# kkahatapitiya/Coarse-Fine-Networks

Hardware: AMD Instinct MI355X
Metric: clips/sec (fwd+bwd+SGD) x3d_fine X3D-M T=256x224x224 (higher is better)
Workload: dtype f32; 1 GPU; x3d_fine X3D-M train step (fwd+loss+bwd+SGD), 8x3x256x224x224 clips per GPU, random-init weights; clips_per_gpu=8, frames=256, parallelism=dp1, launch=eager

## Files before the change

### coarse-fine-networks_amd/cfn_hip/ops.py

```python
import torch
from torch.autograd import Function
from torch.autograd.function import once_differentiable

import ctypes
import threading

from . import call, call_try, check, query, ACT_NONE, ACT_RELU, ACT_SWISH, ACT_SIGMOID


_scratch_epoch = [0]


class _ZeroArena(object):
    CHUNK = 1 << 20

    def __init__(self):
        self.buf, self.off, self.epoch = {}, {}, _scratch_epoch[0]

    def take(self, numel, dev):
        if self.epoch != _scratch_epoch[0]:
            self.buf, self.off, self.epoch = {}, {}, _scratch_epoch[0]
        numel_al = (numel + 1) & ~1
        key = (dev.type, dev.index)
        if key not in self.buf or self.off[key] + numel_al > self.buf[key].numel():
            self.buf[key] = torch.zeros(max(self.CHUNK, numel_al), dtype=torch.float64, device=dev)
            self.off[key] = 0
        o = self.off[key]
        self.off[key] = o + numel_al
        return self.buf[key][o:o + numel]


class _GradCast(object):

    def __init__(self):
        self._reset()
        self.last_total = 0

    def _reset(self):
        self.cur, self.live, self.scheduled, self.seen, self.task = {}, [], False, set(), None

    def begin(self):
        tid = torch._C._current_graph_task_id()
        if tid != self.task:
            if self.live:
                self.flush()
            self._reset()
            self.task = tid

    def first_use(self, w):
        if id(w) in self.seen:
            return False
        self.seen.add(id(w))
        return True

    def take(self, numel, shape, dev):
        al = (numel + 3) & ~3
        key = (dev.type, dev.index)
        ch = self.cur.get(key)
        if ch is None or ch['off'] + al > ch['f64'].numel():
            size = max(int(self.last_total * 1.05) + 1024, al, 1 << 16)
            ch = {'f64': torch.zeros(size, dtype=torch.float64, device=dev),
                  'f32': torch.empty(size, dtype=torch.float32, device=dev), 'off': 0, 'done': 0}
            self.cur[key] = ch
            self.live.append(ch)
        o = ch['off']
        ch['off'] = o + al
        if not self.scheduled:
            torch.autograd.Variable._execution_engine.queue_callback(self._end_of_backward)
            self.scheduled = True
        return ch['f64'][o:o + numel], ch['f32'][o:o + numel].view(shape)

    def flush(self):
        for ch in self.live:
            if ch['off'] > ch['done']:
                ch['f32'][ch['done']:ch['off']].copy_(ch['f64'][ch['done']:ch['off']])
                ch['done'] = ch['off']

    def _end_of_backward(self):
        self.flush()
        self.last_total = max(sum(ch['off'] for ch in self.live), 1)
        self._reset()


class _PerThread(threading.local):

    def __init__(self):
        self.arena = _ZeroArena()
        self.gradcast = _GradCast()


_tls = _PerThread()
LAZY_GRAD_CAST = True


def _f64(n, c, dev):
    return _tls.arena.take(n * c, dev).view(n, c)


def _f64pair(n, c, dev):
    t = _tls.arena.take(2 * n * c, dev).view(2, n, c)
    return t, t[0], t[1]


def reset_scratch():
    _scratch_epoch[0] += 1


def flush_grad_casts():
    _tls.gradcast.flush()


def allow_lazy_grad_cast(params, ok=True):
    for p in params:
        p._cfn_lazy_grad_ok = bool(ok)


def _lazy_ok(w):
    if not LAZY_GRAD_CAST or w is None or not w.is_leaf or w.grad is not None or torch.is_grad_enabled():
        return False
    if not getattr(w, '_cfn_lazy_grad_ok', False):
        return False
    if w._backward_hooks:
        return False
    hooks = getattr(w, '_post_accumulate_grad_hooks', None)
    if hooks:
        from .dist import _BucketHook
        if not all(isinstance(h, _BucketHook) for h in hooks.values()):
            return False
    return True


def _lazy_ok_probe(w):
    with torch.no_grad():
        return _lazy_ok(w)


def _grad_owner(w):
    if w is not None and not w.is_leaf and w._is_view():
        base = w._base
        if base is not None and base.is_leaf and base.numel() == w.numel() and w.is_contiguous() and base.is_contiguous():
            return base
    return w


def _gw_buffers(w, rows, cols, dev):
    gc = _tls.gradcast
    owner = _grad_owner(w)
    if _lazy_ok(owner):
        gc.begin()
        if gc.first_use(owner):
            g64, g32 = gc.take(rows * cols, tuple(w.shape), dev)
            return g64.view(rows, cols), (lambda: g32)
        gc.flush()
    g64 = _f64(rows, cols, dev)
    return g64, (lambda: g64.float().view(tuple(w.shape)))


def _opt(t):
    return None if t is None else t.contiguous()


def _coef(t, rows=None, cols=None):
    if t is None:
        return None
    if rows is not None and t.numel() != rows * cols:
        raise RuntimeError('per-sample coefficients of %d x %d channels expected, got a tensor of shape %s' % (rows, cols, tuple(t.shape)))
    return t.to(torch.float64).contiguous()


class ShortcutToken(object):

    def __init__(self):
        self.acc, self.acc_stride, self.main_done = None, 1, False


class TailLink(object):

    def __init__(self):
        self.y_scale = self.res_scale = None
        self.done = False


def _bf(t):
    return t is not None and t.dtype in (torch.bfloat16, torch.float16)


def subsample_hw(x, s):
    N, C, T, H, W = x.shape
    out = torch.empty(N, C, T, (H - 1) // s + 1, (W - 1) // s + 1, dtype=x.dtype, device=x.device)
    call('cfn_subsample_hw' + _sfx(x), x, out, N * C * T, H, W, s)
    return out


class _PwConv(Function):

    @staticmethod
    def forward(ctx, x, A, B, w, act, stride, want_stats, token, role, tail=None, tail_role=None):
        x = check(x).contiguous()
        N, Cin, T, H, W = x.shape
        Cout = w.shape[0]
        Ho, Wo = (H - 1) // stride + 1, (W - 1) // stride + 1
        y = torch.empty(N, Cout, T, Ho, Wo, dtype=x.dtype, device=x.device)
        s = q = None
        if want_stats:
            s, q = _f64(N, Cout, x.device), _f64(N, Cout, x.device)
        w2 = w.reshape(Cout, Cin).contiguous()
        A, B = _coef(A, N, Cin), _coef(B, N, Cin)
        xs = None
        if _bf(x):
            xs = subsample_hw(x, stride) if stride > 1 else x
            call('cfn_pwconv_fwd' + _sfx(x), xs, A, B, act, w2, y, s, q, N, Cin, Cout, T * Ho * Wo)
        else:
            call('cfn_pwconv_fwd', x, A, B, act, w2, y, s, q, N, Cin, Cout, T, H, W, stride)
        ctx.save_for_backward(x, A, B, w2, y, xs if stride > 1 else None)
        ctx.meta = (act, stride, tuple(w.shape))
        ctx.wparam = w
        ctx.token, ctx.role = token, role
        ctx.tail, ctx.tail_role = tail, tail_role
        if not want_stats:
            return y, None, None
        return y, s, q

    @staticmethod
    @once_differentiable
    def backward(ctx, gy, gs, gq):
        x, A, B, w2, y, xs = ctx.saved_tensors
        act, stride, wshape = ctx.meta
        token, role = ctx.token, ctx.role
        N, Cin, T, H, W = x.shape
        Cout = w2.shape[0]
        gy = torch.zeros_like(y) if gy is None else gy.contiguous()
        gs, gq = _opt(gs), _opt(gq)
        gsc = None
        if ctx.tail is not None and ctx.tail.done:
            gsc = ctx.tail.y_scale if ctx.tail_role == 'y' else ctx.tail.res_scale
        if _bf(x):
            return _PwConv._backward_bf16(ctx, gy, gs, gq, gsc)
        gx = gA = gB = gw = None
        g64 = fin = None
        fused = False
        if ctx.needs_input_grad[0] or (A is not None and ctx.needs_input_grad[1]):
            if token is not None and role == 'short' and stride > 1 and not token.main_done:
                Ho, Wo = y.shape[3], y.shape[4]
                da = torch.empty(N, Cin, T, Ho, Wo, dtype=torch.float32, device=x.device)
                call('cfn_pwconv_bwd_data_acc', gy, y, gs, gq, w2, None, None, None, ACT_NONE, da, None, None, N, Cin, Cout, T,
                     Ho, Wo, 1, None, 1, gsc)
                token.acc, token.acc_stride = da, stride
            else:
                gx = torch.zeros_like(x) if stride != 1 else torch.empty_like(x)
                ab = a64 = b64 = None
                if A is not None:
                    ab, a64, b64 = _f64pair(N, Cin, x.device)
                acc, acc_stride = None, 1
                if token is not None and role == 'main':
                    if token.acc is not None:
                        acc, acc_stride, token.acc = token.acc, token.acc_stride, None
                    else:
                        token.main_done = True
                if stride == 1 and ctx.needs_input_grad[3]:
                    g64, fin = _gw_buffers(ctx.wparam, Cout, Cin, x.device)
                    fused = call_try('cfn_pwconv_bwd_fused', gy, y, gs, gq, w2, x, A, B, act, gx, a64, b64, g64, N, Cin, Cout,
                                     T, H, W, acc, acc_stride, gsc)
                if not fused:
                    call('cfn_pwconv_bwd_data_acc', gy, y, gs, gq, w2, x, A, B, act, gx, a64, b64, N, Cin, Cout, T, H, W, stride,
                         acc, acc_stride, gsc)
                if A is not None:
                    gA, gB = ab[0], ab[1]
        if ctx.needs_input_grad[3]:
            if g64 is None:
                g64, fin = _gw_buffers(ctx.wparam, Cout, Cin, x.device)
            if not fused:
                call('cfn_pwconv_bwd_weight', gy, y, gs, gq, x, A, B, act, g64, N, Cin, Cout, T, H, W, stride, gsc)
            gw = fin()
        return gx, gA, gB, gw, None, None, None, None, None, None, None

    @staticmethod
    def _backward_bf16(ctx, gy, gs, gq, gsc):
        x, A, B, w2, y, xs = ctx.saved_tensors
        act, stride, wshape = ctx.meta
        token, role = ctx.token, ctx.role
        N, Cin, T, H, W = x.shape
        Cout = w2.shape[0]
        Ho, Wo = y.shape[3], y.shape[4]
        xin = xs if stride > 1 else x
        gx = gA = gB = gw = None
        if ctx.needs_input_grad[0] or (A is not None and ctx.needs_input_grad[1]):
            if token is not None and role == 'short' and stride > 1 and not token.main_done:
                da = torch.empty(N, Cin, T, Ho, Wo, dtype=x.dtype, device=x.device)
                call('cfn_pwconv_bwd_data' + _sfx(gy), gy, y, gs, gq, w2, None, None, None, ACT_NONE, da, None, None, N, Cin, Cout, T,
                     Ho, Wo, None, 1, gsc)
                token.acc, token.acc_stride = da, stride
            else:
                ab = a64 = b64 = None
                if A is not None:
                    ab, a64, b64 = _f64pair(N, Cin, x.device)
                acc, acc_stride = None, 1
                if token is not None and role == 'main':
                    if token.acc is not None:
                        acc, acc_stride, token.acc = token.acc, token.acc_stride, None
                    else:
                        token.main_done = True
                gxc = torch.empty_like(xin)
                call('cfn_pwconv_bwd_data' + _sfx(gy), gy, y, gs, gq, w2, xin, A, B, act, gxc, a64, b64, N, Cin, Cout, T, Ho, Wo,
                     acc, acc_stride, gsc)
                if stride > 1:
                    gx = torch.zeros_like(x)
                    gx[:, :, :, ::stride, ::stride] = gxc
                else:
                    gx = gxc
                if A is not None:
                    gA, gB = ab[0], ab[1]
        if ctx.needs_input_grad[3]:
            g64, fin = _gw_buffers(ctx.wparam, Cout, Cin, x.device)
            call('cfn_pwconv_bwd_weight' + _sfx(gy), gy, y, gs, gq, xin, A, B, act, g64, N, Cin, Cout, T * Ho * Wo, gsc)
            gw = fin()
        return gx, gA, gB, gw, None, None, None, None, None, None, None


def pwconv(x, w, A=None, B=None, act=ACT_NONE, stride=1, stats=True, token=None, role=None, tail=None, tail_role=None):
    N, Cin, T, H, W = x.shape
    Ho, Wo = (H - 1) // stride + 1, (W - 1) // stride + 1
    es = x.element_size()
    lim = (1 << 31) if es == 4 else (1 << 30)
    span = max(Cin * H * W, w.shape[0] * H * W, w.shape[0] * Ho * Wo, Cin * Ho * Wo) * es
    needs_grad = torch.is_grad_enabled() and any(t is not None and t.requires_grad for t in (x, w, A, B))
    if span * T < lim or needs_grad or T == 1:
        return _PwConv.apply(x, A, B, w, act, stride, stats, token, role, tail, tail_role)
    step = max((lim - 1) // span, 1)
    odd_plane = es == 2 and (Ho * Wo) % 2 == 1
    if odd_plane:
        if 2 * span >= lim:
            raise RuntimeError('pwconv: two frames of %d x %d x %d bf16 elements exceed the 1 GiB buffer range the frame-range '
                               'chunking has to respect (odd plane: frames travel in pairs)' % (max(Cin, w.shape[0]), H, W))
        step = max(step & ~1, 2)
    y = torch.empty(N, w.shape[0], T, Ho, Wo, dtype=x.dtype, device=x.device)
    s = q = None
    t0 = 0
    while t0 < T:
        t1 = min(t0 + step, T)
        if odd_plane and (t1 - t0) % 2 and t1 - t0 > 1:
            t1 -= 1
        pad = odd_plane and (t1 - t0) % 2 == 1
        xc = x[:, :, t0:t1].contiguous()
        if pad:
            xc = torch.cat([xc, torch.zeros_like(xc)], 2)
        yc, sc, qc = _PwConv.apply(xc, A, B, w, act, stride, False if pad else stats, None, None)
        if pad:
            yc = yc[:, :, :1]
            if stats:
                sc, qc = yc.double().sum((2, 3, 4)), (yc.double() ** 2).sum((2, 3, 4))
        y[:, :, t0:t1] = yc
        if stats:
            s, q = (sc, qc) if s is None else (s + sc, q + qc)
        t0 = t1
    return y, s, q


def _sfx(t):
    return '_bf16' if t.dtype == torch.bfloat16 else ('_f16' if t.dtype == torch.float16 else '')


class _DwConv3d(Function):

    @staticmethod
    def forward(ctx, x, A, B, w, act, stride, want_stats):
        x = check(x).contiguous()
        N, C, T, H, W = x.shape
        Ho, Wo = (H + 2 - 3) // stride + 1, (W + 2 - 3) // stride + 1
        y = torch.empty(N, C, T, Ho, Wo, dtype=x.dtype, device=x.device)
        s = q = None
        if want_stats:
            s, q = _f64(N, C, x.device), _f64(N, C, x.device)
        w2 = w.reshape(C, 27).contiguous()
        A, B = _coef(A, N, C), _coef(B, N, C)
        call('cfn_dwconv3d_fwd' + _sfx(x), x, A, B, act, w2, y, s, q, N, C, T, H, W, stride)
        ctx.save_for_backward(x, A, B, w2, y)
        ctx.meta = (act, stride, tuple(w.shape))
        ctx.wparam = w
        if not want_stats:
            return y, None, None
        return y, s, q

    @staticmethod
    @once_differentiable
    def backward(ctx, gy, gs, gq):
        x, A, B, w2, y = ctx.saved_tensors
        act, stride, wshape = ctx.meta
        N, C, T, H, W = x.shape
        gy = torch.zeros_like(y) if gy is None else gy.contiguous()
        gs, gq = _opt(gs), _opt(gq)
        gx = gA = gB = gw = None
        want_x = ctx.needs_input_grad[0] or (A is not None and ctx.needs_input_grad[1])
        want_w = ctx.needs_input_grad[3]
        ab = a64 = b64 = g64 = fin = None
        if want_x:
            gx = torch.empty_like(x)
            if A is not None:
                ab, a64, b64 = _f64pair(N, C, x.device)
        if want_w:
            g64, fin = _gw_buffers(ctx.wparam, C, 27, x.device)
        sfx = _sfx(x)
        fused = want_x and want_w and stride == 1 and call_try('cfn_dwconv3d_bwd_fused' + sfx, gy, y, gs, gq, w2, x, A, B, act,
                                                             gx, a64, b64, g64, N, C, T, H, W)
        if not fused and want_x and want_w and stride == 2:
            fused = call_try('cfn_dwconv3d_bwd_fused_s2' + sfx, gy, y, gs, gq, w2, x, A, B, act, gx, a64, b64, g64, N, C, T, H, W)
        if not fused:
            if want_x:
                call('cfn_dwconv3d_bwd_data' + sfx, gy, y, gs, gq, w2, x, A, B, act, gx, a64, b64, N, C, T, H, W, stride)
            if want_w:
                call('cfn_dwconv3d_bwd_weight' + sfx, gy, y, gs, gq, x, A, B, act, g64, N, C, T, H, W, stride)
        if want_x and A is not None:
            gA, gB = ab[0], ab[1]
        if want_w:
            gw = fin()
        return gx, gA, gB, gw, None, None, None


def dwconv3d(x, w, A=None, B=None, act=ACT_NONE, stride=1, stats=True):
    return _DwConv3d.apply(x, A, B, w, act, stride, stats)


class _DwConvT5(Function):

    @staticmethod
    def forward(ctx, x, w, want_stats, out_dtype=None):
        x = check(x, torch.float32).contiguous()
        N, C, T, H, W = x.shape
        y = torch.empty_like(x, dtype=out_dtype or x.dtype)
        s = q = None
        if want_stats:
            s, q = _f64(N, C, x.device), _f64(N, C, x.device)
        w2 = w.reshape(C, 5).contiguous()
        call('cfn_dwconv_t5_fwd' + _sfx(y), x, w2, y, s, q, N, C, T, H * W)
        ctx.save_for_backward(x, w2, y)
        ctx.wshape = tuple(w.shape)
        ctx.wparam = w
        if not want_stats:
            return y, None, None
        return y, s, q

    @staticmethod
    @once_differentiable
    def backward(ctx, gy, gs, gq):
        x, w2, y = ctx.saved_tensors
        N, C, T, H, W = x.shape
        gy = torch.zeros_like(y) if gy is None else gy.contiguous()
        gs, gq = _opt(gs), _opt(gq)
        gx = gw = None
        want_x, want_w = ctx.needs_input_grad[0], ctx.needs_input_grad[1]
        if want_x:
            gx = torch.empty_like(x)
        if want_w:
            g64, fin = _gw_buffers(ctx.wparam, C, 5, x.device)
        fused = want_x and want_w and call_try('cfn_dwconv_t5_bwd_fused' + _sfx(y), gy, y, gs, gq, w2, x, gx, g64, N, C, T, H * W)
        if not fused:
            if want_x:
                call('cfn_dwconv_t5_bwd_data' + _sfx(y), gy, y, gs, gq, w2, gx, N, C, T, H * W)
            if want_w:
                call('cfn_dwconv_t5_bwd_weight' + _sfx(y), gy, y, gs, gq, x, g64, N, C, T, H * W)
        if want_w:
            gw = fin()
        return gx, gw, None, None


def dwconv_t5(x, w, stats=True, out_dtype=None):
    return _DwConvT5.apply(x, w, stats, out_dtype)


class _StemConv(Function):

    @staticmethod
    def forward(ctx, x, w):
        x = check(x).contiguous()
        N, Ci, T, H, W = x.shape
        Co = w.shape[0]
        Ho, Wo = (H + 2 - 3) // 2 + 1, (W + 2 - 3) // 2 + 1
        y = torch.empty(N, Co, T, Ho, Wo, dtype=torch.float32, device=x.device)
        w2 = w.reshape(Co, Ci * 9).contiguous()
        call('cfn_stem_conv_fwd', x, w2, y, N, Ci, Co, T, H, W)
        ctx.save_for_backward(x)
        ctx.wshape = tuple(w.shape)
        ctx.wparam = w
        return y

    @staticmethod
    @once_differentiable
    def backward(ctx, gy):
        (x,) = ctx.saved_tensors
        N, Ci, T, H, W = x.shape
        Co = ctx.wshape[0]
        gw = None
        if ctx.needs_input_grad[1]:
            g64, fin = _gw_buffers(ctx.wparam, Co, Ci * 9, x.device)
            call('cfn_stem_conv_bwd_weight', gy.contiguous(), x, g64, N, Ci, Co, T, H, W)
            gw = fin()
        return None, gw


def stem_conv(x, w):
    return _StemConv.apply(x, w)


from .u8clips import clip_lut


def _u8_args(frames, lengths, lut):
    if frames.dtype != torch.uint8 or frames.dim() != 5 or frames.shape[4] != 3:
        raise RuntimeError('uint8 frames of shape (N, T, H, W, 3) expected, got %s %s' % (frames.dtype, tuple(frames.shape)))
    if lut.dtype != torch.float32 or lut.numel() != 3 * 256:
        raise RuntimeError('a (3, 256) fp32 table expected (ops.clip_lut), got %s %s' % (lut.dtype, tuple(lut.shape)))
    if lengths is not None:
        if lengths.numel() != frames.shape[0]:
            raise RuntimeError('one length per clip expected: %d clips, lengths %s' % (frames.shape[0], tuple(lengths.shape)))
        lengths = lengths.to(torch.int32).contiguous()
    return frames.contiguous(), lengths, lut.contiguous()


def clip_u8_to_f32(frames, lut, lengths=None):
    frames, lengths, lut = _u8_args(frames, lengths, lut)
    N, T, H, W, _ = frames.shape
    x = torch.empty(N, 3, T, H, W, dtype=torch.float32, device=frames.device)
    call('cfn_clip_u8_to_f32', frames, lut, lengths, x, N, T, H, W)
    return x


class _StemConvU8(Function):

    @staticmethod
    def forward(ctx, frames, lengths, lut, w):
        frames, lengths, lut = _u8_args(frames, lengths, lut)
        N, T, H, W, Ci = frames.shape
        Co = w.shape[0]
        Ho, Wo = (H + 2 - 3) // 2 + 1, (W + 2 - 3) // 2 + 1
        y = torch.empty(N, Co, T, Ho, Wo, dtype=torch.float32, device=frames.device)
        w2 = w.reshape(Co, Ci * 9).contiguous()
        if not call_try('cfn_stem_conv_u8_fwd', frames, lut, lengths, w2, y, N, Ci, Co, T, H, W):
            call('cfn_stem_conv_fwd', clip_u8_to_f32(frames, lut, lengths), w2, y, N, Ci, Co, T, H, W)
        ctx.save_for_backward(frames, lengths, lut)
        ctx.wshape = tuple(w.shape)
        ctx.wparam = w
        return y

    @staticmethod
    @once_differentiable
    def backward(ctx, gy):
        frames, lengths, lut = ctx.saved_tensors
        N, T, H, W, Ci = frames.shape
        Co = ctx.wshape[0]
        gw = None
# ... 723 lines not shown
```

### include/cfn_hip.h

```cpp
#ifndef CFN_HIP_H
#define CFN_HIP_H
#ifdef __cplusplus
extern "C" {
#endif

const char* cfn_last_error(void);
const char* cfn_version(void);
int cfn_device_info(int* cus, int* lds_per_cu, char* name, int name_len);

int cfn_prof_enable(int family, int on);
int cfn_prof_collect(int family, double* total_ms, long* launches, double* total_bytes);

int cfn_dwconv3d_fwd(const float* x, const double* A, const double* B, int act, const float* w, float* y, double* sum,
                     double* sumsq, int N, int C, int T, int Hi, int Wi, int stride, void* stream);
int cfn_dwconv3d_bwd_data(const float* gy, const float* y, const double* gsum, const double* gsumsq, const float* w,
                          const float* x, const double* A, const double* B, int act, float* gx, double* gA, double* gB,
                          int N, int C, int T, int Hi, int Wi, int stride, void* stream);
int cfn_dwconv3d_bwd_weight(const float* gy, const float* y, const double* gsum, const double* gsumsq, const float* x,
                            const double* A, const double* B, int act, double* gw, int N, int C, int T, int Hi, int Wi,
                            int stride, void* stream);
int cfn_dwconv3d_bwd_fused(const float* gy, const float* y, const double* gsum, const double* gsumsq, const float* w,
                           const float* x, const double* A, const double* B, int act, float* gx, double* gA, double* gB,
                           double* gw, int N, int C, int T, int H, int W, void* stream);
int cfn_dwconv3d_bwd_fused_s2(const float* gy, const float* y, const double* gsum, const double* gsumsq, const float* w,
                              const float* x, const double* A, const double* B, int act, float* gx, double* gA, double* gB,
                              double* gw, int N, int C, int T, int H, int W, void* stream);

int cfn_dwconv_t5_fwd(const float* x, const float* w, float* y, double* sum, double* sumsq, int N, int C, int T,
                      long plane, void* stream);
int cfn_dwconv_t5_bwd_data(const float* gy, const float* y, const double* gsum, const double* gsumsq, const float* w,
                           float* gx, int N, int C, int T, long plane, void* stream);
int cfn_dwconv_t5_bwd_weight(const float* gy, const float* y, const double* gsum, const double* gsumsq, const float* x,
                             double* gw, int N, int C, int T, long plane, void* stream);
int cfn_dwconv_t5_bwd_fused(const float* gy, const float* y, const double* gsum, const double* gsumsq, const float* w,
                            const float* x, float* gx, double* gw, int N, int C, int T, long plane, void* stream);

int cfn_pwconv_fwd(const float* x, const double* A, const double* B, int act, const float* w, float* y, double* sum,
                   double* sumsq, int N, int Cin, int Cout, int T, int Hi, int Wi, int stride, void* stream);
int cfn_pwconv_bwd_data(const float* gy, const float* y, const double* gsum, const double* gsumsq, const float* w,
                        const float* x, const double* A, const double* B, int act, float* gx, double* gA, double* gB, int N,
                        int Cin, int Cout, int T, int Hi, int Wi, int stride, void* stream);
int cfn_pwconv_bwd_data_acc(const float* gy, const float* y, const double* gsum, const double* gsumsq, const float* w,
                        const float* x, const double* A, const double* B, int act, float* gx, double* gA, double* gB, int N,
                        int Cin, int Cout, int T, int Hi, int Wi, int stride, const float* acc, int acc_stride,
                        const double* gscale, void* stream);
int cfn_pwconv_bwd_weight(const float* gy, const float* y, const double* gsum, const double* gsumsq, const float* x,
                          const double* A, const double* B, int act, double* gw, int N, int Cin, int Cout, int T, int Hi,
                          int Wi, int stride, const double* gscale, void* stream);

int cfn_pw_split_terms(int terms);

int cfn_deterministic(int on);

int cfn_pwconv_bwd_fused(const float* gy, const float* y, const double* gsum, const double* gsumsq, const float* w,
                         const float* x, const double* A, const double* B, int act, float* gx, double* gA, double* gB,
                         double* gw, int N, int Cin, int Cout, int T, int Hi, int Wi, const float* acc, int acc_stride,
                         const double* gscale, void* stream);

int cfn_stem_conv_fwd(const float* x, const float* w, float* y, int N, int Cimg, int Cout, int T, int Hi, int Wi,
                      void* stream);
int cfn_stem_conv_bwd_weight(const float* gy, const float* x, double* gw, int N, int Cimg, int Cout, int T, int Hi, int Wi,
                             void* stream);

int cfn_clip_u8_to_f32(const unsigned char* frames, const float* lut, const int* lengths, float* x, int N, int T, int H, int W,
                       void* stream);
int cfn_stem_conv_u8_fwd(const unsigned char* frames, const float* lut, const int* lengths, const float* w, float* y, int N,
                         int Cimg, int Cout, int T, int Hi, int Wi, void* stream);
int cfn_stem_conv_u8_bwd_weight(const float* gy, const unsigned char* frames, const float* lut, const int* lengths, double* gw,
                                int N, int Cimg, int Cout, int T, int Hi, int Wi, void* stream);

int cfn_bn_fold_fwd(const double* s, const double* q, const float* gamma, const float* beta, float* run_mean, float* run_var,
                    long* nbt, int training, int N, int C, int S, double count, double eps, double momentum, const float* w1,
                    const float* b1, const float* w2, const float* b2, int Wd, double pool_count, double* A, double* B,
                    double* mean, double* rstd, float* A0, float* B0, float* gate, float* hbuf, float* pooled, void* stream);
int cfn_bn_fold_bwd(const double* gA, const double* gB, const double* s, const float* gamma, const double* mean,
                    const double* rstd, const float* A0, const float* B0, const float* gate, const float* hbuf,
                    const float* pooled, const float* w1, const float* w2, int training, int N, int C, int S, int Wd,
                    double count, double pool_count, double* gs, double* gq, float* ggamma, float* gbeta, float* gw1,
                    float* gb1, float* gw2, float* gb2, double* tA, double* tB, void* stream);

int cfn_conv3d_dense_fwd(const float* x, const double* A, const double* B, int act, const float* w, float* y, double* sum,
                         double* sumsq, int N, int Cin, int Cout, int T, int Hi, int Wi, const int* geom, void* stream);
int cfn_conv3d_dense_bwd_data(const float* gy, const float* y, const double* gsum, const double* gsumsq, const float* w,
                              const float* x, const double* A, const double* B, int act, float* gx, double* gA, double* gB,
                              int N, int Cin, int Cout, int T, int Hi, int Wi, const int* geom, void* stream);
int cfn_conv3d_dense_bwd_weight(const float* gy, const float* y, const double* gsum, const double* gsumsq, const float* x,
                                const double* A, const double* B, int act, double* gw, int N, int Cin, int Cout, int T, int Hi,
                                int Wi, const int* geom, void* stream);

int cfn_gauss_align_fwd(const long* meta, const float* mask, const float* gx, double tx, double ratio, float* GX, int B, int crops,
                        int Tf, int K, void* stream);
int cfn_gauss_align_bwd(const float* gGX, const long* meta, const float* mask, const float* gx, double tx, double ratio,
                        float* ggx, int B, int crops, int Tf, int K, void* stream);

int cfn_fusion_gather_fwd(const float* x, const float* at_raw, const float* at_bias, const float* GX, const float* mask, float* z,
                          float* den, int B, int crops, int C, int Tf, int K, int P, void* stream);
int cfn_fusion_gather_bwd(const float* gz, const float* z, const float* den, const float* x, const float* at_raw,
                          const float* at_bias, const float* GX, const float* mask, float* gx, float* gat, float* gGX, float* dw,
                          int B, int crops, int C, int Tf, int K, int P, void* stream);

int cfn_bn_add_relu_fwd(const float* y, const double* A, const double* B, const float* res, const double* Ar, const double* Br,
                        float* out, int* mask, long NC, long vol, void* stream);
int cfn_bn_add_relu_bwd(const float* gout, const float* gout2, const float* out, const float* y, const double* A, const float* res,
                        const double* Ar, float* gy, float* gres, double* gA, double* gB, double* gAr, long NC, long vol,
                        void* stream);
long cfn_bn_add_relu_mask_words(long NC, long vol);
int cfn_bn_add_relu_bwd_g(const float* gout, const float* gout2, const float* out, const int* mask, const float* y,
                          const float* res, float* g, double* gA, double* gB, double* gAr, long NC, long vol, void* stream);

int cfn_affine_act_fwd(const float* x, const double* A, const double* B, int act, float* out, long NC, long vol, void* stream);
int cfn_affine_act_bwd(const float* gout, const float* x, const double* A, const double* B, int act, float* gx, double* gA,
                       double* gB, long NC, long vol, void* stream);
int cfn_channel_stats(const float* x, double* sum, double* sumsq, long NC, long vol, void* stream);

int cfn_pool_hw_fwd(const float* x, const double* A, const double* B, int act, float* out, long NC, int T, int H, int W, int OH,
                    int OW, void* stream);
int cfn_pool_hw_bwd(const float* gout, const float* x, const double* A, const double* B, int act, float* gx, double* gA,
                    double* gB, long NC, int T, int H, int W, int OH, int OW, void* stream);

int cfn_film_fwd(const float* x, const float* m, const float* c, float* out, long NC, int T, int H, int W, int f,
                 void* stream);
int cfn_film_bwd(const float* g, const float* x, const float* m, float* gx, float* gm, float* gc, long NC, int T, int H,
                 int W, int f, void* stream);

int cfn_grid_time_index(const float* cdf, int n, int Tin, int* i0, float* w1, void* stream);
int cfn_grid_cdf_fwd(const float* g, const float* bias, float* cdf, int B, int Kin, void* stream);
int cfn_grid_cdf_bwd(const float* gcdf, const float* g, const float* bias, float* gg, int B, int Kin, void* stream);
int cfn_time_sample_fwd(const float* x, const float* cdf, float* out, int B, int C, int Tin, int K, long P, void* stream);
int cfn_time_sample_bwd(const float* g, const float* x, const float* cdf, float* gx, double* gcdf, int B, int C, int Tin,
                        int K, long P, void* stream);

int cfn_time_pool_fwd(const float* x, float* out, int mode, long BC, int Tin, int R, long P, void* stream);
int cfn_time_pool_bwd(const float* g, const float* x, float* gx, int mode, long BC, int Tin, int R, long P, void* stream);

int cfn_interp1d_fwd(const float* x, const float* y, const float* xnew, float* ynew, long* ind, int B, int N, int Pq,
                     int xrow, int yrow, int qrow, void* stream);
int cfn_interp1d_bwd(const float* g, const float* x, const float* y, const float* xnew, const long* ind, float* gx, float* gy,
                     float* gq, int B, int N, int Pq, int xrow, int yrow, int qrow, void* stream);

int cfn_time_resize_fwd(const float* x, float* out, long BC, int Kin, int Lout, long P, int align_corners, void* stream);
int cfn_time_resize_bwd(const float* g, float* gx, long BC, int Kin, int Lout, long P, int align_corners, void* stream);

int cfn_detloss_fwd(const float* logits, const float* labels, const float* masks, const float* norm, double world, float* probs,
                    float* cls, float* loc, int* jstar, float* ymax, double* rows, double* norm_used, int B, int C, int T, int TL,
                    int n, int align_corners, void* stream);
int cfn_detloss_bwd(const float* g_cls, const float* g_loc, const float* logits, const float* labels, const float* masks,
                    const int* jstar, const float* ymax, const double* norm_used, double world, float* gx, int B, int C, int T,
                    int TL, int n, int align_corners, void* stream);

int cfn_pwconv_fwd_bf16(const unsigned short* x, const double* A, const double* B, int act, const float* w, unsigned short* y,
                        double* sum, double* sumsq, int N, int Cin, int Cout, long Q, void* stream);
int cfn_pwconv_bwd_data_bf16(const unsigned short* gy, const unsigned short* y, const double* gsum, const double* gsumsq,
                             const float* w, const unsigned short* x, const double* A, const double* B, int act,
                             unsigned short* gx, double* gA, double* gB, int N, int Cin, int Cout, int T, int H, int W,
                             const unsigned short* acc, int acc_stride, const double* gscale, void* stream);
int cfn_pwconv_bwd_weight_bf16(const unsigned short* gy, const unsigned short* y, const double* gsum, const double* gsumsq,
                               const unsigned short* x, const double* A, const double* B, int act, double* gw, int N, int Cin,
                               int Cout, long Q, const double* gscale, void* stream);
int cfn_subsample_hw_bf16(const unsigned short* x, unsigned short* out, long planes, int H, int W, int s, void* stream);

int cfn_dwconv3d_fwd_bf16(const unsigned short* x, const double* A, const double* B, int act, const float* w, unsigned short* y,
                          double* sum, double* sumsq, int N, int C, int T, int Hi, int Wi, int stride, void* stream);
int cfn_dwconv3d_bwd_data_bf16(const unsigned short* gy, const unsigned short* y, const double* gsum, const double* gsumsq,
                               const float* w, const unsigned short* x, const double* A, const double* B, int act,
                               unsigned short* gx, double* gA, double* gB, int N, int C, int T, int Hi, int Wi, int stride,
                               void* stream);
int cfn_dwconv3d_bwd_weight_bf16(const unsigned short* gy, const unsigned short* y, const double* gsum, const double* gsumsq,
                                 const unsigned short* x, const double* A, const double* B, int act, double* gw, int N, int C,
                                 int T, int Hi, int Wi, int stride, void* stream);
int cfn_dwconv3d_bwd_fused_bf16(const unsigned short* gy, const unsigned short* y, const double* gsum, const double* gsumsq,
                                const float* w, const unsigned short* x, const double* A, const double* B, int act,
                                unsigned short* gx, double* gA, double* gB, double* gw, int N, int C, int T, int H, int W,
                                void* stream);
int cfn_dwconv3d_bwd_fused_s2_bf16(const unsigned short* gy, const unsigned short* y, const double* gsum, const double* gsumsq,
                                   const float* w, const unsigned short* x, const double* A, const double* B, int act,
                                   unsigned short* gx, double* gA, double* gB, double* gw, int N, int C, int T, int H, int W,
                                   void* stream);

int cfn_dwconv_t5_fwd_bf16(const float* x, const float* w, unsigned short* y, double* sum, double* sumsq, int N, int C, int T,
                           long plane, void* stream);
int cfn_dwconv_t5_bwd_data_bf16(const unsigned short* gy, const unsigned short* y, const double* gsum, const double* gsumsq,
                                const float* w, float* gx, int N, int C, int T, long plane, void* stream);
int cfn_dwconv_t5_bwd_weight_bf16(const unsigned short* gy, const unsigned short* y, const double* gsum, const double* gsumsq,
                                  const float* x, double* gw, int N, int C, int T, long plane, void* stream);
int cfn_dwconv_t5_bwd_fused_bf16(const unsigned short* gy, const unsigned short* y, const double* gsum, const double* gsumsq,
                                 const float* w, const float* x, float* gx, double* gw, int N, int C, int T, long plane,
                                 void* stream);

long cfn_bn_add_relu_mask_words_bf16(long NC, long vol);
int cfn_bn_add_relu_fwd_bf16(const unsigned short* y, const double* A, const double* B, const unsigned short* res,
                             const double* Ar, const double* Br, unsigned short* out, int* mask, long NC, long vol, void* stream);
int cfn_bn_add_relu_bwd_g_bf16(const unsigned short* gout, const unsigned short* gout2, const unsigned short* out, const int* mask,
                               const unsigned short* y, const unsigned short* res, unsigned short* g, double* gA, double* gB,
                               double* gAr, long NC, long vol, void* stream);
int cfn_pool_hw_fwd_bf16(const unsigned short* x, const double* A, const double* B, int act, float* out, long NC, int T, int H,
                         int W, int OH, int OW, void* stream);
int cfn_pool_hw_bwd_bf16(const float* gout, const unsigned short* x, const double* A, const double* B, int act,
                         unsigned short* gx, double* gA, double* gB, long NC, int T, int H, int W, int OH, int OW, void* stream);

int cfn_pwconv_fwd_f16(const unsigned short* x, const double* A, const double* B, int act, const float* w, unsigned short* y,
                        double* sum, double* sumsq, int N, int Cin, int Cout, long Q, void* stream);
int cfn_pwconv_bwd_data_f16(const unsigned short* gy, const unsigned short* y, const double* gsum, const double* gsumsq,
                             const float* w, const unsigned short* x, const double* A, const double* B, int act,
                             unsigned short* gx, double* gA, double* gB, int N, int Cin, int Cout, int T, int H, int W,
                             const unsigned short* acc, int acc_stride, const double* gscale, void* stream);
int cfn_pwconv_bwd_weight_f16(const unsigned short* gy, const unsigned short* y, const double* gsum, const double* gsumsq,
                               const unsigned short* x, const double* A, const double* B, int act, double* gw, int N, int Cin,
                               int Cout, long Q, const double* gscale, void* stream);
int cfn_subsample_hw_f16(const unsigned short* x, unsigned short* out, long planes, int H, int W, int s, void* stream);

int cfn_dwconv3d_fwd_f16(const unsigned short* x, const double* A, const double* B, int act, const float* w, unsigned short* y,
                          double* sum, double* sumsq, int N, int C, int T, int Hi, int Wi, int stride, void* stream);
int cfn_dwconv3d_bwd_data_f16(const unsigned short* gy, const unsigned short* y, const double* gsum, const double* gsumsq,
                               const float* w, const unsigned short* x, const double* A, const double* B, int act,
                               unsigned short* gx, double* gA, double* gB, int N, int C, int T, int Hi, int Wi, int stride,
                               void* stream);
int cfn_dwconv3d_bwd_weight_f16(const unsigned short* gy, const unsigned short* y, const double* gsum, const double* gsumsq,
                                 const unsigned short* x, const double* A, const double* B, int act, double* gw, int N, int C,
                                 int T, int Hi, int Wi, int stride, void* stream);
int cfn_dwconv3d_bwd_fused_f16(const unsigned short* gy, const unsigned short* y, const double* gsum, const double* gsumsq,
                                const float* w, const unsigned short* x, const double* A, const double* B, int act,
                                unsigned short* gx, double* gA, double* gB, double* gw, int N, int C, int T, int H, int W,
                                void* stream);
int cfn_dwconv3d_bwd_fused_s2_f16(const unsigned short* gy, const unsigned short* y, const double* gsum, const double* gsumsq,
                                   const float* w, const unsigned short* x, const double* A, const double* B, int act,
                                   unsigned short* gx, double* gA, double* gB, double* gw, int N, int C, int T, int H, int W,
                                   void* stream);

int cfn_dwconv_t5_fwd_f16(const float* x, const float* w, unsigned short* y, double* sum, double* sumsq, int N, int C, int T,
                           long plane, void* stream);
int cfn_dwconv_t5_bwd_data_f16(const unsigned short* gy, const unsigned short* y, const double* gsum, const double* gsumsq,
                                const float* w, float* gx, int N, int C, int T, long plane, void* stream);
int cfn_dwconv_t5_bwd_weight_f16(const unsigned short* gy, const unsigned short* y, const double* gsum, const double* gsumsq,
                                  const float* x, double* gw, int N, int C, int T, long plane, void* stream);
int cfn_dwconv_t5_bwd_fused_f16(const unsigned short* gy, const unsigned short* y, const double* gsum, const double* gsumsq,
                                 const float* w, const float* x, float* gx, double* gw, int N, int C, int T, long plane,
                                 void* stream);

long cfn_bn_add_relu_mask_words_f16(long NC, long vol);
int cfn_bn_add_relu_fwd_f16(const unsigned short* y, const double* A, const double* B, const unsigned short* res,
                             const double* Ar, const double* Br, unsigned short* out, int* mask, long NC, long vol, void* stream);
int cfn_bn_add_relu_bwd_g_f16(const unsigned short* gout, const unsigned short* gout2, const unsigned short* out, const int* mask,
                               const unsigned short* y, const unsigned short* res, unsigned short* g, double* gA, double* gB,
                               double* gAr, long NC, long vol, void* stream);
int cfn_pool_hw_fwd_f16(const unsigned short* x, const double* A, const double* B, int act, float* out, long NC, int T, int H,
                         int W, int OH, int OW, void* stream);
int cfn_pool_hw_bwd_f16(const float* gout, const unsigned short* x, const double* A, const double* B, int act,
                         unsigned short* gx, double* gA, double* gB, long NC, int T, int H, int W, int OH, int OW, void* stream);

int cfn_crop_resize_flip_u8(const unsigned char* src, const int* lengths, const int* box, const int* bounds, const int* coef,
                            unsigned char* dst, int N, int T, int Hs, int Ws, int S, int K, void* stream);

int cfn_ap_append(const float* probs, const float* labels, const int* valid, float* scores, unsigned char* targets, int* count,
                  int* flags, int B, int K, int TL, long cap, void* stream);
int cfn_ap_sort(const float* scores, const unsigned char* targets, const int* count, float* sorted_scores,
                unsigned char* sorted_targets, int* tmp_keys, unsigned char* tmp_targets, int K, long cap, void* stream);
int cfn_ap_reduce(const unsigned char* sorted_targets, const int* count, float* ap, int K, long cap, void* stream);
int cfn_ap_sort_tile(void);

#ifdef __cplusplus
}
#endif
#endif
```

Measured before the change: 104.2 clips/s.

## Fuse strided shortcut pointwise-conv backward data and weight grads into one kernel

Adds a HIP kernel for the stride-2 shortcut 1x1x1 conv backward. It computes the data gradient (stored into the accumulation buffer for the main branch) and the weight gradient in a single pass over gy/y and the strided input, using MFMA tiles and a double-buffered LDS pipeline. This removes the separate data-grad and weight-grad launches and the repeated reads of gy. The cost is extra register and LDS pressure, plus FP64 atomics for the weight gradient, and it falls back to the old path for unsupported shapes.

```diff
diff --git a/coarse-fine-networks_amd/cfn_hip/ops.py b/coarse-fine-networks_amd/cfn_hip/ops.py
--- a/coarse-fine-networks_amd/cfn_hip/ops.py
+++ b/coarse-fine-networks_amd/cfn_hip/ops.py
@@ -243,8 +243,13 @@
             if token is not None and role == 'short' and stride > 1 and not token.main_done:
                 Ho, Wo = y.shape[3], y.shape[4]
                 da = torch.empty(N, Cin, T, Ho, Wo, dtype=torch.float32, device=x.device)
-                call('cfn_pwconv_bwd_data_acc', gy, y, gs, gq, w2, None, None, None, ACT_NONE, da, None, None, N, Cin, Cout, T,
-                     Ho, Wo, 1, None, 1, gsc)
+                if ctx.needs_input_grad[3]:
+                    g64, fin = _gw_buffers(ctx.wparam, Cout, Cin, x.device)
+                    fused = call_try('cfn_pwconv_short_bwd', gy, y, gs, gq, gsc, w2, x, A, B, act, da, g64, N, Cin, Cout, T, H, W,
+                                     stride)
+                if not fused:
+                    call('cfn_pwconv_bwd_data_acc', gy, y, gs, gq, w2, None, None, None, ACT_NONE, da, None, None, N, Cin, Cout, T,
+                         Ho, Wo, 1, None, 1, gsc)
                 token.acc, token.acc_stride = da, stride
             else:
                 gx = torch.zeros_like(x) if stride != 1 else torch.empty_like(x)
diff --git a/coarse-fine-networks_amd/csrc/pwshort.hip b/coarse-fine-networks_amd/csrc/pwshort.hip
--- /dev/null
+++ b/coarse-fine-networks_amd/csrc/pwshort.hip
@@ -0,0 +1,303 @@
+#include "cfn_common.h"
+#include <stdlib.h>
+
+#include "pw_common.h"
+
+typedef float __attribute__((ext_vector_type(4))) sf4;
+
+
+struct PshArgs {
+    const float* gy; const float* y; const double* gs; const double* gq; const double* gsc;
+    const float* w;
+    const float* x; const double* pa; const double* pb;
+    float* da; double* gw;
+    int N, M, K, Q, P;
+    int HiWi, Wi, HoWo, Wo, nstrips, stages;
+};
+
+template <int MT, int NT, int KT16, int KS, int WM, int WP, int PSH_PT, int VEC, int ACT, int OCC>
+__global__ __launch_bounds__(64 * WM * WP, OCC) void pw_short_bwd_kernel(const PshArgs a) {
+    extern __shared__ __attribute__((aligned(16))) float smem[];
+    constexpr int NTHR = 64 * WM * WP, PSH_PITCH = PSH_PT + 1;
+    constexpr int BM = 32 * MT, BN = 32 * NT;
+    constexpr int MTW = MT / WM, NTW16 = KT16 / WM;
+    constexpr int PW = PSH_PT / WP, NGRP = PW / 16;
+    constexpr int GTR = PSH_PT / 4, XTR = PSH_PT / 2;
+    constexpr int GRS = NTHR / GTR, NG = (BM + GRS - 1) / GRS;
+    constexpr int XRS = NTHR / XTR, NX = (16 * KT16 + XRS - 1) / XRS;
+    static_assert(MT % WM == 0 && KT16 % WM == 0 && PSH_PT % (16 * WP) == 0 && 4 * KS <= BM && 16 * KT16 <= BN, "tile split");
+    const int tid = threadIdx.x, lane = tid & 63, half = lane >> 5, col = lane & 31;
+    const int wave = cfn_uni(tid >> 6), wm = wave / WP, wp = wave - wm * WP;
+    const int m16 = lane & 15, kq = lane >> 4;
+    const unsigned L = cfn_xcd_remap(blockIdx.x, gridDim.x);
+    const int strip = L % a.nstrips;
+    const int n = L / a.nstrips;
+    const int M = a.M, K = a.K, Q = a.Q;
+
+    constexpr int IMG = (BM + BN) * PSH_PITCH;
+    float* img0 = smem;
+    float* sCg = smem + 2 * IMG;
+    float* sCz = sCg + 2 * BM;
+    for (int e = tid; e < 2 * IMG; e += NTHR) smem[e] = 0.0f;
+    for (int m = tid; m < BM; m += NTHR) {
+        const bool ok = m < M;
+        sCg[2 * m] = (ok && a.gs) ? (float)a.gs[(long)n * M + m] : 0.0f;
+        sCg[2 * m + 1] = (ok && a.gq && a.y) ? 2.0f * (float)a.gq[(long)n * M + m] : 0.0f;
+        sCz[m] = (ok && a.gsc) ? (float)a.gsc[(long)n * M + m] : 1.0f;
+    }
+    float wq[NTW16][KS];
+#pragma unroll
+    for (int t = 0; t < NTW16; ++t)
+#pragma unroll
+        for (int s = 0; s < KS; ++s) {
+            const int ci = (wm * NTW16 + t) * 16 + m16, co = 4 * s + kq;
+            wq[t][s] = (ci < K && co < M) ? a.w[(long)co * K + ci] : 0.0f;
+        }
+    float ca[NT], cb[NT];
+#pragma unroll
+    for (int j = 0; j < NT; ++j) {
+        const int k = j * 32 + col;
+        const bool ok = a.pa != nullptr && k < K;
+        ca[j] = ok ? (float)a.pa[(long)n * K + k] : 1.0f;
+        cb[j] = ok ? (float)a.pb[(long)n * K + k] : 0.0f;
+    }
+    f16v acc[MTW][NT];
+#pragma unroll
+    for (int i = 0; i < MTW; ++i)
+#pragma unroll
+        for (int j = 0; j < NT; ++j)
+#pragma unroll
+            for (int r = 0; r < 16; ++r) acc[i][j][r] = 0.0f;
+    __syncthreads();
+
+    constexpr int OOB = 0x7ffffff0;
+    __amdgpu_buffer_rsrc_t rg = cfn_rsrc(const_cast<float*>(a.gy + (long)n * M * Q), (unsigned)((long)M * Q * 4));
+    __amdgpu_buffer_rsrc_t ry = cfn_rsrc(const_cast<float*>((a.y ? a.y : a.gy) + (long)n * M * Q), a.y ? (unsigned)((long)M * Q * 4) : 0u);
+    __amdgpu_buffer_rsrc_t rx = cfn_rsrc(const_cast<float*>(a.x + (long)n * K * a.P), (unsigned)((long)K * a.P * 4));
+    __amdgpu_buffer_rsrc_t rd = cfn_rsrc(a.da + (long)n * K * Q, (unsigned)((long)K * Q * 4));
+    const int lrow = tid / GTR, c4 = (tid % GTR) * 4;
+    const int xrow = tid / XTR, pp = (tid % XTR) * 2;
+    sf4 pg[NG], py[NG];
+    float px0[NX], px1[NX];
+    int vog[NG], vox[NX];
+#pragma unroll
+    for (int it = 0; it < NG; ++it) vog[it] = (it * GRS + lrow) < M ? ((it * GRS + lrow) * Q + c4) * 4 : OOB;
+#pragma unroll
+    for (int it = 0; it < NX; ++it) vox[it] = (it * XRS + xrow) < K ? (it * XRS + xrow) * a.P * 4 : OOB;
+    auto xlat = [&](int q) {
+        const int t = q / a.HoWo, r = q - t * a.HoWo;
+        const int oh = r / a.Wo, ow = r - oh * a.Wo;
+        return t * a.HiWi + 2 * oh * a.Wi + 2 * ow;
+    };
+    auto prefetch = [&](int q0) {
+        if (VEC >= 1) {
+            const bool inq = q0 + c4 < Q;
+#pragma unroll
+            for (int it = 0; it < NG; ++it) {
+                const int vo = inq ? vog[it] : OOB;
+                pg[it] = __builtin_bit_cast(sf4, __builtin_amdgcn_raw_buffer_load_b128(rg, vo, q0 * 4, 0));
+                py[it] = __builtin_bit_cast(sf4, __builtin_amdgcn_raw_buffer_load_b128(ry, vo, q0 * 4, 0));
+            }
+        } else {
+#pragma unroll
+            for (int it = 0; it < NG; ++it) {
+#pragma unroll
+                for (int e = 0; e < 4; ++e) {
+                    const int vo = (q0 + c4 + e < Q && vog[it] != OOB) ? vog[it] + 4 * e : OOB;
+                    pg[it][e] = pw_bload(rg, vo, q0 * 4);
+                    py[it][e] = pw_bload(ry, vo, q0 * 4);
+                }
+            }
+        }
+        const int qx = q0 + pp;
+        if (VEC == 2) {
+            const int xo = qx < Q ? xlat(qx) * 4 : OOB;
+#pragma unroll
+            for (int it = 0; it < NX; ++it) {
+                const sf4 v = __builtin_bit_cast(sf4, __builtin_amdgcn_raw_buffer_load_b128(rx, (xo == OOB || vox[it] == OOB) ? OOB : vox[it] + xo, 0, 0));
+                px0[it] = v.x; px1[it] = v.z;
+            }
+        } else {
+            const int xo0 = qx < Q ? xlat(qx) * 4 : OOB;
+            const int xo1 = qx + 1 < Q ? xlat(qx + 1) * 4 : OOB;
+#pragma unroll
+            for (int it = 0; it < NX; ++it) {
+                px0[it] = pw_bload(rx, (xo0 == OOB || vox[it] == OOB) ? OOB : vox[it] + xo0, 0);
+                px1[it] = pw_bload(rx, (xo1 == OOB || vox[it] == OOB) ? OOB : vox[it] + xo1, 0);
+            }
+        }
+    };
+    auto stage = [&](int q0, float* sG, float* sX) {
+#pragma unroll
+        for (int it = 0; it < NG; ++it) {
+            const int row = it * GRS + lrow;
+            if (NG * GRS > BM && row >= BM) continue;
+            const float cs = cfn_settle(sCg[2 * row]), cq = cfn_settle(sCg[2 * row + 1]), cz = cfn_settle(sCz[row]);
+            const bool rok = row < M;
+            float* d = sG + row * PSH_PITCH + c4;
+#pragma unroll
+            for (int e = 0; e < 4; ++e) d[e] = (rok && q0 + c4 + e < Q) ? fmaf(py[it][e], cq, fmaf(pg[it][e], cz, cs)) : 0.0f;
+        }
+#pragma unroll
+        for (int it = 0; it < NX; ++it) {
+            const int row = it * XRS + xrow;
+            if (NX * XRS > 16 * KT16 && row >= 16 * KT16) continue;
+            float* d = sX + row * PSH_PITCH + pp;
+            d[0] = px0[it]; d[1] = px1[it];
+        }
+    };
+
+    const int qbeg = strip * a.stages * PSH_PT;
+    const int nst = min(a.stages, (Q - qbeg + PSH_PT - 1) / PSH_PT);
+    if (nst > 0) {
+        prefetch(qbeg);
+        stage(qbeg, img0, img0 + BM * PSH_PITCH);
+        if (nst > 1) prefetch(qbeg + PSH_PT);
+    }
+    __syncthreads();
+    const int pbase = wp * PW;
+    for (int st = 0; st < nst; ++st) {
+        const int q0 = qbeg + st * PSH_PT;
+        float* cur = img0 + (st & 1) * IMG;
+        float* nxt = img0 + ((st + 1) & 1) * IMG;
+        if (st + 1 < nst) {
+            stage(q0 + PSH_PT, nxt, nxt + BM * PSH_PITCH);
+            if (st + 2 < nst) prefetch(q0 + 2 * PSH_PT);
+        }
+        const float* sG = cur;
+        const float* sX = cur + BM * PSH_PITCH;
+#pragma unroll
+        for (int s = 0; s < PW / 2; ++s) {
+            const int p = pbase + 2 * s + half;
+            float av[MTW], bv[NT];
+#pragma unroll
+            for (int i = 0; i < MTW; ++i) av[i] = sG[((wm * MTW + i) * 32 + col) * PSH_PITCH + p];
+#pragma unroll
+            for (int j = 0; j < NT; ++j) {
+                const float xr = cfn_settle(sX[(j * 32 + col) * PSH_PITCH + p]);
+                bv[j] = cfn_act<ACT>(fmaf(xr, ca[j], cb[j]));
+            }
+#pragma unroll
+            for (int i = 0; i < MTW; ++i)
+#pragma unroll
+                for (int j = 0; j < NT; ++j) acc[i][j] = __builtin_amdgcn_mfma_f32_32x32x2f32(av[i], bv[j], acc[i][j], 0, 0, 0);
+            if ((s & 3) == 3) __builtin_amdgcn_sched_barrier(0);
+        }
+        sf4 dv[NGRP][NTW16];
+#pragma unroll
+        for (int g = 0; g < NGRP; ++g)
+#pragma unroll
+            for (int t = 0; t < NTW16; ++t) dv[g][t] = (sf4){0.f, 0.f, 0.f, 0.f};
+#pragma unroll
+        for (int s = 0; s < KS; ++s) {
+#pragma unroll
+            for (int g = 0; g < NGRP; ++g) {
+                const float b = sG[(4 * s + kq) * PSH_PITCH + pbase + 16 * g + m16];
+#pragma unroll
+                for (int t = 0; t < NTW16; ++t) dv[g][t] = __builtin_amdgcn_mfma_f32_16x16x4f32(wq[t][s], b, dv[g][t], 0, 0, 0);
+            }
+            if ((s & 3) == 3) __builtin_amdgcn_sched_barrier(0);
+        }
+#pragma unroll
+        for (int g = 0; g < NGRP; ++g) {
+            const int pl = pbase + 16 * g + m16;
+            const bool qv = q0 + pl < Q;
+#pragma unroll
+            for (int t = 0; t < NTW16; ++t) {
+                const sf4 v = dv[g][t];
+                const float ve[4] = {v.x, v.y, v.z, v.w};
+#pragma unroll
+                for (int r = 0; r < 4; ++r) {
+                    const int ci = (wm * NTW16 + t) * 16 + 4 * kq + r;
+                    __builtin_amdgcn_raw_buffer_store_b32(__builtin_bit_cast(unsigned, ve[r]), rd, (qv && ci < K) ? (ci * Q + pl) * 4 : OOB,
+                                                          q0 * 4, 0);
+                }
+            }
+        }
+        __syncthreads();
+    }
+
+    constexpr int CWP = BN + 1;
+    float* cw = smem + wp * (BM * CWP);
+#pragma unroll
+    for (int i = 0; i < MTW; ++i)
+#pragma unroll
+        for (int j = 0; j < NT; ++j)
+#pragma unroll
+            for (int r = 0; r < 16; ++r) {
+                const int ml = (wm * MTW + i) * 32 + (r & 3) + 8 * (r >> 2) + 4 * half;
+                cw[ml * CWP + j * 32 + col] = acc[i][j][r];
+            }
+    __syncthreads();
+    for (int e = tid; e < BM * BN; e += NTHR) {
+        const int ml = e / BN, kl = e - ml * BN;
+        const int o = ml * CWP + kl;
+        float v = smem[o];
+#pragma unroll
+        for (int p = 1; p < WP; ++p) v += smem[p * BM * CWP + o];
+        if (ml < M && kl < K) cfn_add64(&a.gw[(long)ml * K + kl], (double)v);
+    }
+}
+
+template <int MT, int NT, int KT16, int KS, int WM, int WP, int PSH_PT, int OCC>
+static int psh_launch(PshArgs& a, int act, int vec, hipStream_t st) {
+    constexpr int BM = 32 * MT, BN = 32 * NT, PSH_PITCH = PSH_PT + 1;
+    size_t lds = ((size_t)2 * (BM + BN) * PSH_PITCH + 3 * BM) * sizeof(float);
+    const size_t lds_cw = (size_t)WP * BM * (BN + 1) * sizeof(float);
+    if (lds_cw > lds) lds = lds_cw;
+    const long nst = cfn_cdiv(a.Q, PSH_PT);
+    const long slots = 256L * OCC;
+    const long rounds = (nst * a.N >= slots * 2 * 16) ? 2 : 1;
+    long want = slots * rounds / a.N;
+    if (want < 1) want = 1;
+    long stages = cfn_cdiv(nst, want);
+    if (stages < 4) stages = 4;
+    a.stages = (int)stages;
+    a.nstrips = cfn_cdiv(nst, stages);
+    const unsigned blocks = (unsigned)((long)a.N * a.nstrips);
+#define CFN_PSH_GO(VECV, ACTV)                                                                                  \
+    do {                                                                                                        \
+        auto k = pw_short_bwd_kernel<MT, NT, KT16, KS, WM, WP, PSH_PT, VECV, ACTV, OCC>;                                \
+        if (lds > 48 * 1024) (void)hipFuncSetAttribute((const void*)k, hipFuncAttributeMaxDynamicSharedMemorySize, (int)lds); \
+        hipLaunchKernelGGL(k, dim3(blocks), dim3(64 * WM * WP), lds, st, a);                                    \
+    } while (0)
+    const bool relu = act == CFN_ACT_RELU;
+    if (vec == 2) { if (relu) CFN_PSH_GO(2, CFN_ACT_RELU); else CFN_PSH_GO(2, CFN_ACT_NONE); }
+    else if (vec == 1) { if (relu) CFN_PSH_GO(1, CFN_ACT_RELU); else CFN_PSH_GO(1, CFN_ACT_NONE); }
+    else { if (relu) CFN_PSH_GO(0, CFN_ACT_RELU); else CFN_PSH_GO(0, CFN_ACT_NONE); }
+#undef CFN_PSH_GO
+    return cfn_check_launch("pwconv_short_bwd");
+}
+
+extern "C" int cfn_pwconv_short_bwd(const float* gy, const float* y, const double* gsum, const double* gsumsq, const double* gscale,
+                                    const float* w, const float* x, const double* A, const double* B, int act, float* da, double* gw,
+                                    int N, int Cin, int Cout, int T, int Hi, int Wi, int stride, void* stream) {
+    CFN_REQUIRE(gy && w && x && da && gw, "cfn_pwconv_short_bwd: null tensor");
+    CFN_REQUIRE((A == nullptr) == (B == nullptr), "cfn_pwconv_short_bwd: A/B mismatch");
+    CFN_REQUIRE(gsumsq == nullptr || y != nullptr, "cfn_pwconv_short_bwd: gsumsq needs y");
+    CFN_REQUIRE(N > 0 && Cin > 0 && Cout > 0 && T > 0 && Hi > 0 && Wi > 0 && stride >= 1, "cfn_pwconv_short_bwd: bad shape");
+    if (stride != 2) return -1;
+    { const char* e = getenv("CFN_PW_SHORT"); if (e && e[0] && atoi(e) == 0) return -1; }
+    if (A && act != CFN_ACT_NONE && act != CFN_ACT_RELU) return -1;
+    if (Cout > 192 || Cin > 96) return -1;
+    const int Ho = (Hi - 1) / 2 + 1, Wo = (Wi - 1) / 2 + 1;
+    const long Ql = (long)T * Ho * Wo, Pl = (long)T * Hi * Wi;
+    const int big = Cout > Cin ? Cout : Cin;
+    if ((long)big * Pl * 4 >= 0x7ffffff0L || N > 65535) return -1;
+    if ((((uintptr_t)gy | (uintptr_t)x | (uintptr_t)da | (uintptr_t)(y ? y : gy)) & 3) != 0) return -1;
+    const bool gvec = Ql % 4 == 0 && (((uintptr_t)gy | (uintptr_t)(y ? y : gy)) & 15) == 0;
+    const bool xvec = Wo % 2 == 0 && Wi % 2 == 0 && ((long)Hi * Wi) % 4 == 0 && ((uintptr_t)x & 15) == 0;
+    const int vec = gvec ? (xvec ? 2 : 1) : 0;
+    PshArgs a = {};
+    a.gy = gy; a.y = gsumsq ? y : nullptr; a.gs = gsum; a.gq = gsumsq; a.gsc = gscale; a.w = w; a.x = x; a.pa = A; a.pb = B;
+    a.da = da; a.gw = gw;
+    a.N = N; a.M = Cout; a.K = Cin; a.Q = (int)Ql; a.P = (int)Pl;
+    a.HiWi = Hi * Wi; a.Wi = Wi; a.HoWo = Ho * Wo; a.Wo = Wo;
+    const int pact = A ? act : CFN_ACT_NONE;
+    hipStream_t st = (hipStream_t)stream;
+    CfnProfScope prof(CFN_K_PWCONV_BWD, st, 4.0 * N * ((double)Cout * Ql * (a.y ? 2 : 1) + (double)Cin * Ql * 3));
+    if (Cout <= 24 && Cin <= 32) return psh_launch<1, 1, 2, 6, 1, 4, 64, 3>(a, pact, vec, st);
+    if (Cout <= 48 && Cin <= 32) return psh_launch<2, 1, 2, 12, 1, 4, 64, 2>(a, pact, vec, st);
+    if (Cout <= 96 && Cin <= 48) return psh_launch<3, 2, 3, 24, 3, 2, 64, 1>(a, pact, vec, st);
+    return psh_launch<6, 3, 6, 48, 6, 1, 32, 1>(a, pact, vec, st);
+}
diff --git a/include/cfn_hip.h b/include/cfn_hip.h
--- a/include/cfn_hip.h
+++ b/include/cfn_hip.h
@@ -56,6 +56,10 @@
                          const float* x, const double* A, const double* B, int act, float* gx, double* gA, double* gB,
                          double* gw, int N, int Cin, int Cout, int T, int Hi, int Wi, const float* acc, int acc_stride,
                          const double* gscale, void* stream);
+
+int cfn_pwconv_short_bwd(const float* gy, const float* y, const double* gsum, const double* gsumsq, const double* gscale,
+                         const float* w, const float* x, const double* A, const double* B, int act, float* da, double* gw,
+                         int N, int Cin, int Cout, int T, int Hi, int Wi, int stride, void* stream);
 
 int cfn_stem_conv_fwd(const float* x, const float* w, float* y, int N, int Cimg, int Cout, int T, int Hi, int Wi,
                       void* stream);
```

Measured after the change: 105.6 clips/s (median of 6 runs). 1.4% higher.
